# mit-han-lab/litepose

Measured on AMD Instinct MI355X. Metric: images/sec end-to-end (backbone+deconv+AE-group), LitePose-XS@256 b64, higher is better.
Workload: dtype f32

## Files before the change

litepose_amd/csrc/net_kernels.hip:

```cpp
#include "kernels.h"
#include "split3.h"

#include <cstdio>
#include <cstdlib>
#include <type_traits>
#include <utility>

namespace lp {

thread_local const char* last_kernel_tag = "";
thread_local LaunchNote last_launch;
thread_local bool launch_notes = false;

void note_launch(const void* fn, dim3 grid, dim3 block, size_t lds) {
    int per_cu = 0;
    const int threads = (int)(block.x * block.y * block.z);
    if (hipOccupancyMaxActiveBlocksPerMultiprocessor(&per_cu, fn, threads, lds) != hipSuccess) per_cu = 0;
    last_launch.grid = (int)((long)grid.x * grid.y * grid.z);
    last_launch.block = threads;
    last_launch.lds = (int)lds;
    last_launch.wgs_per_cu = per_cu;
}

typedef float f32x4 __attribute__((ext_vector_type(4)));
// ... 2234 lines not shown
        if (!mbconv2 || !wrow || !w1s || Cout > 16) return false;
        const size_t lds2 = (size_t)16 * MB3_PAIR * sizeof(float);
        last_kernel_tag = "mbconv2_kernel";
#define LP_MB2(RESV)                                                                                       \
        do {                                                                                               \
            if (uses_scratch(reinterpret_cast<const void*>(mbconv2_kernel<RESV, 8, 1>))) return false;     \
            static bool attr2_##RESV = false;                                                              \
            if (!attr2_##RESV) {                                                                           \
                (void)hipFuncSetAttribute(reinterpret_cast<const void*>(mbconv2_kernel<RESV, 8, 1>),       \
                                          hipFuncAttributeMaxDynamicSharedMemorySize, (int)lds2);          \
                attr2_##RESV = true;                                                                       \
            }                                                                                              \
            LP_LAUNCH((mbconv2_kernel<RESV, 8, 1>), grid, block, lds2, s, x, (const f32x4*)wrow,  \
                               (const u32x4*)w1s, b1f, w2p, b2f, out, Cin, Cexp, Cout, H, W, tilesX, tilesY, \
                               xcd_remap_mode());                                                          \
        } while (0)
        if (res) LP_MB2(true); else LP_MB2(false);
#undef LP_MB2
        return true;
    }
    const size_t lds = (size_t)(16 * MB2_PAIR) * sizeof(float);
    last_kernel_tag = "mbconv_kernel";
#define LP_MB(RESV)                                                                                        \
    do {                                                                                                   \
        if (uses_scratch(reinterpret_cast<const void*>(mbconv_kernel<RESV, 12, false, false>))) return false; \
        static bool attr_##RESV = false;                                                                   \
        if (!attr_##RESV) {                                                                                \
            (void)hipFuncSetAttribute(reinterpret_cast<const void*>(mbconv_kernel<RESV, 12, false, false>), \
                                      hipFuncAttributeMaxDynamicSharedMemorySize, (int)lds);               \
            attr_##RESV = true;                                                                            \
        }                                                                                                  \
        LP_LAUNCH((mbconv_kernel<RESV, 12, false, false>), grid, block, lds, s, x, (const f32x4*)nullptr, \
                           (const u32x4*)nullptr, w1p, b1f, wdw_pair, bdw, w2p, b2f, out, Cin, Cexp, Cout, H, W, \
                           tilesX, tilesY, xcd_remap_mode());                                              \
    } while (0)
    if (res) LP_MB(true); else LP_MB(false);
#undef LP_MB
    return true;
}

template <int COT, bool DUAL>
__global__ __launch_bounds__(256) void deconv_pair_kernel(const float* __restrict__ inA, int Ca,
                                                          const float* __restrict__ inB, int Cb,
                                                          const float* __restrict__ w,
                                                          const float* __restrict__ b,
                                                          float* __restrict__ out, int N, int h,
                                                          int w_, int Cout) {
    const long total = (long)N * h * w_;
    const long g = (long)blockIdx.x * blockDim.x + threadIdx.x;
    if (g >= total) return;
    const int ix = (int)(g % w_);
    const int iy = (int)((g / w_) % h);
    const int n = (int)(g / ((long)w_ * h));
    const int co0 = blockIdx.y * COT;
    float acc[COT][4];
#pragma unroll
    for (int c = 0; c < COT; ++c) acc[c][0] = acc[c][1] = acc[c][2] = acc[c][3] = 0.f;

    for (int src = 0; src < (DUAL ? 2 : 1); ++src) {
        const float* in = src == 0 ? inA : inB;
        const int Cs = src == 0 ? Ca : Cb;
        const int cbase = src == 0 ? 0 : Ca;
        for (int ci = 0; ci < Cs; ++ci) {
            const float* plane = in + ((long)n * Cs + ci) * h * w_;
            float v[3][3];
#pragma unroll
            for (int dy = -1; dy <= 1; ++dy)
#pragma unroll
                for (int dx = -1; dx <= 1; ++dx) {
                    const int y = iy + dy, x = ix + dx;
                    v[dy + 1][dx + 1] =
                        (y >= 0 && y < h && x >= 0 && x < w_) ? plane[(long)y * w_ + x] : 0.f;
                }
            const float* wc = w + ((long)(cbase + ci) * Cout + co0) * 16;
#pragma unroll
            for (int c = 0; c < COT; ++c) {
                if (co0 + c < Cout) {
                    const float* k = wc + c * 16;
#pragma unroll
                    for (int a = 0; a < 2; ++a)
#pragma unroll
                        for (int bb = 0; bb < 2; ++bb) {
                            const int dy0 = a == 0 ? 0 : 1, ky0 = a == 0 ? 1 : 0;
                            const int dy1 = a == 0 ? -1 : 0, ky1 = a == 0 ? 3 : 2;
                            const int dx0 = bb == 0 ? 0 : 1, kx0 = bb == 0 ? 1 : 0;
                            const int dx1 = bb == 0 ? -1 : 0, kx1 = bb == 0 ? 3 : 2;
                            float t = acc[c][a * 2 + bb];
                            t = fmaf(v[dy0 + 1][dx0 + 1], k[ky0 * 4 + kx0], t);
                            t = fmaf(v[dy0 + 1][dx1 + 1], k[ky0 * 4 + kx1], t);
                            t = fmaf(v[dy1 + 1][dx0 + 1], k[ky1 * 4 + kx0], t);
                            t = fmaf(v[dy1 + 1][dx1 + 1], k[ky1 * 4 + kx1], t);
                            acc[c][a * 2 + bb] = t;
                        }
                }
            }
        }
    }
    const int OW = 2 * w_, OH = 2 * h;
#pragma unroll
    for (int c = 0; c < COT; ++c) {
        const int co = co0 + c;
        if (co < Cout) {
            const float bias = b[co];
            float* o = out + ((long)n * Cout + co) * OH * OW + (long)(2 * iy) * OW + 2 * ix;
            float2 r0 = {fmaxf(acc[c][0] + bias, 0.f), fmaxf(acc[c][1] + bias, 0.f)};
            float2 r1 = {fmaxf(acc[c][2] + bias, 0.f), fmaxf(acc[c][3] + bias, 0.f)};
            *reinterpret_cast<float2*>(o) = r0;
            *reinterpret_cast<float2*>(o + OW) = r1;
        }
    }
}

template <bool DUAL>
__global__ __launch_bounds__(256) void deconv_mfma_kernel(const float* __restrict__ inA, int Ca,
                                                          const float* __restrict__ inB, int Cb,
                                                          const float* __restrict__ wp,
                                                          const float* __restrict__ bias,
                                                          float* __restrict__ out, long NP, int h, int w_,
                                                          int Cout) {
    const int lane = threadIdx.x & 63;
    const int wave = threadIdx.x >> 6;
    const long px0 = ((long)blockIdx.x * 4 + wave) * 32;
    if (px0 >= NP) return;
    const int half = lane >> 5, pl = lane & 31;
    const long g = px0 + pl;
    const bool valid = g < NP;
    const long gc = valid ? g : NP - 1;
    const int hw = h * w_;
    const int n = (int)(gc / hw);
    const int p = (int)(gc - (long)n * hw);
    const int iy = p / w_, ix = p - iy * w_;
    const int par = blockIdx.y, a = par >> 1, b = par & 1;
    const int Ct = DUAL ? Ca + Cb : Ca;
    const int KP = 2 * Ct;
    int toff[4];
    bool tok[4];
#pragma unroll
    for (int t = 0; t < 4; ++t) {
        const int tyi = t >> 1, txi = t & 1;
        const int dy = a == 0 ? (tyi == 0 ? 0 : -1) : (tyi == 0 ? 1 : 0);
        const int dx = b == 0 ? (txi == 0 ? 0 : -1) : (txi == 0 ? 1 : 0);
        const int y = iy + dy, x = ix + dx;
        tok[t] = y >= 0 && y < h && x >= 0 && x < w_;
        toff[t] = tok[t] ? y * w_ + x : p;
    }
    f32x16 acc;
#pragma unroll
    for (int r = 0; r < 16; ++r) acc[r] = 0.f;
    const f32x4* bp = reinterpret_cast<const f32x4*>(bias + half * 16);
    f32x4 bfr[4];
#pragma unroll
    for (int q = 0; q < 4; ++q) bfr[q] = bp[q];
    const float* wl = wp + (long)par * KP * 64 + lane;
    int kbase = 0;
#pragma unroll
    for (int t = 0; t < 4; ++t) {
#pragma unroll 1
        for (int srcsel = 0; srcsel < (DUAL ? 2 : 1); ++srcsel) {
            const int C = srcsel == 0 ? Ca : Cb;
            const float* sp = (srcsel == 0 ? inA : inB) + ((long)n * C + half) * hw + toff[t];
            const int nkp = C >> 1;
#pragma unroll 8
            for (int kp = 0; kp < nkp; ++kp) {
                float bv = sp[(long)(2 * kp) * hw];
                bv = tok[t] ? bv : 0.f;
                const float av = wl[(long)(kbase + kp) * 64];
                acc = __builtin_amdgcn_mfma_f32_32x32x2f32(av, bv, acc, 0, 0, 0);
            }
            kbase += nkp;
        }
    }
    if (!valid) return;
    const int OW = 2 * w_;
    float* ob = out + (long)n * Cout * 4 * hw + (long)(2 * iy + a) * OW + 2 * ix + b;
#pragma unroll
    for (int r = 0; r < 16; ++r) {
        const int co = 4 * half + (r & 3) + 8 * (r >> 2);
        if (co < Cout) ob[(long)co * 4 * hw] = fmaxf(acc[r] + bfr[r >> 2][r & 3], 0.f);
    }
}

template <int NB, bool DUAL>
__global__ __launch_bounds__(256) void deconv4_kernel(const float* __restrict__ inA, int Ca,
                                                      const float* __restrict__ inB, int Cb,
                                                      const f32x4* __restrict__ wq,
                                                      const float* __restrict__ bias,
                                                      float* __restrict__ out, long NP, int h, int w_,
                                                      int Cout, int xcd_remap) {
    const int lane = threadIdx.x & 63;
    const int wave = threadIdx.x >> 6;
    const int bid = xcd_remap ? xcd_contiguous_id(blockIdx.x, gridDim.x) : blockIdx.x;
    const long px0 = ((long)bid * 4 + wave) * 32;
    if (px0 >= NP) return;
    const int half = lane >> 5, pl = lane & 31;
    const long g = px0 + pl;
    const bool valid = g < NP;
    const long gc = valid ? g : NP - 1;
    const int hw = h * w_;
    const int n = (int)(gc / hw);
    const int p = (int)(gc - (long)n * hw);
    const int iy = p / w_, ix = p - iy * w_;
    int voff[9];
    bool vok[9];
#pragma unroll
    for (int v = 0; v < 9; ++v) {
        const int y = iy + v / 3 - 1, x = ix + v % 3 - 1;
        vok[v] = y >= 0 && y < h && x >= 0 && x < w_;
        voff[v] = vok[v] ? y * w_ + x : p;
    }
    f32x16 acc[NB][4];
#pragma unroll
    for (int i = 0; i < NB; ++i)
#pragma unroll
        for (int q = 0; q < 4; ++q)
#pragma unroll
            for (int r = 0; r < 16; ++r) acc[i][q][r] = 0.f;
    f32x4 bfr[NB][4];
#pragma unroll
    for (int i = 0; i < NB; ++i) {
        const f32x4* bp = reinterpret_cast<const f32x4*>(bias + (i * 2 + half) * 16);
#pragma unroll
        for (int q = 0; q < 4; ++q) bfr[i][q] = bp[q];
    }
    const int CP = (DUAL ? Ca + Cb : Ca) >> 1, CPA = Ca >> 1;
    const f32x4* wl = wq + lane;
    const float* spA = inA + ((long)n * Ca + half) * hw;
    const float* spB = DUAL ? inB + ((long)n * Cb + half) * hw : spA;
    auto fetch = [&](int cp, float (&bv)[9], f32x4 (&av)[NB][4]) {
        const int c = min(cp, CP - 1);
        const float* cpn = (!DUAL || c < CPA) ? spA + (long)(2 * c) * hw : spB + (long)(2 * (c - CPA)) * hw;
#pragma unroll
        for (int v = 0; v < 9; ++v) bv[v] = cpn[voff[v]];
#pragma unroll
        for (int i = 0; i < NB; ++i)
#pragma unroll
            for (int q = 0; q < 4; ++q) av[i][q] = wl[((long)(i * 4 + q) * CP + c) * 64];
    };
    auto mma = [&](const float (&raw)[9], const f32x4 (&av)[NB][4]) {
        float bv[9];
#pragma unroll
        for (int v = 0; v < 9; ++v) bv[v] = vok[v] ? raw[v] : 0.f;
#pragma unroll
        for (int t = 0; t < 4; ++t) {
            const int tyi = t >> 1, txi = t & 1;
#pragma unroll
            for (int i = 0; i < NB; ++i)
#pragma unroll
                for (int q = 0; q < 4; ++q) {
                    const int a = q >> 1, b = q & 1;
                    const int dy = a == 0 ? (tyi == 0 ? 0 : -1) : (tyi == 0 ? 1 : 0);
                    const int dx = b == 0 ? (txi == 0 ? 0 : -1) : (txi == 0 ? 1 : 0);
                    acc[i][q] = __builtin_amdgcn_mfma_f32_32x32x2f32(av[i][q][t], bv[(dy + 1) * 3 + dx + 1], acc[i][q],
                                                                     0, 0, 0);
                }
        }
    };
    float bv0[9], bv1[9];
    f32x4 av0[NB][4], av1[NB][4];
    fetch(0, bv0, av0);
#pragma unroll 1
    for (int cp = 0; cp < CP; cp += 2) {
        fetch(cp + 1, bv1, av1);
        __builtin_amdgcn_sched_barrier(0);
        mma(bv0, av0);
        __builtin_amdgcn_sched_barrier(0);
        fetch(cp + 2, bv0, av0);
        __builtin_amdgcn_sched_barrier(0);
        mma(bv1, av1);
        __builtin_amdgcn_sched_barrier(0);
    }
    if (!valid) return;
    const int OW = 2 * w_;
    float* ob = out + (long)n * Cout * 4 * hw + (long)(2 * iy) * OW + 2 * ix;
#pragma unroll
    for (int i = 0; i < NB; ++i)
#pragma unroll
        for (int r = 0; r < 16; ++r) {
            const int co = i * 32 + 4 * half + (r & 3) + 8 * (r >> 2);
            if (co < Cout) {
                const float bb = bfr[i][r >> 2][r & 3];
                float* o = ob + (long)co * 4 * hw;
                const float2 top = {fmaxf(acc[i][0][r] + bb, 0.f), fmaxf(acc[i][1][r] + bb, 0.f)};
                const float2 bot = {fmaxf(acc[i][2][r] + bb, 0.f), fmaxf(acc[i][3][r] + bb, 0.f)};
                *reinterpret_cast<float2*>(o) = top;
                *reinterpret_cast<float2*>(o + OW) = bot;
            }
        }
}

void launch_deconv4(const float* inA, int Ca, const float* inB, int Cb, const float* wq, const float* bias,
                    float* out, int N, int h, int w_, int Cout, hipStream_t s) {
    const long NP = (long)N * h * w_;
    dim3 grid((unsigned)((NP + 127) / 128)), block(256);
#define LP_D4(NBV, DV) LP_LAUNCH((deconv4_kernel<NBV, DV>), grid, block, 0, s, inA, Ca, inB, Cb, (const f32x4*)wq, bias, \
                                 out, NP, h, w_, Cout, xcd_remap_mode())
    if (inB) { if (Cout <= 32) LP_D4(1, true); else LP_D4(2, true); }
    else { if (Cout <= 32) LP_D4(1, false); else LP_D4(2, false); }
#undef LP_D4
    last_kernel_tag = "deconv4_kernel";
}


struct D4X3 {
    __host__ __device__ static constexpr int twl(int w) { return w <= 16 ? 4 : 5; }
    __host__ __device__ static constexpr int rows(int twl) { return 4 * (32 >> twl); }
    __host__ __device__ static constexpr int rs(int twl) { return twl == 5 ? 34 : 32; }
    __host__ __device__ static constexpr int cells(int twl) { return (rows(twl) + 2) * rs(twl); }
    __host__ __device__ static constexpr int slab_groups(int twl) { return twl == 5 ? 6 : 4; }
    static constexpr int REC = 48;
};

struct D4Prod { int v, q, t; };
__host__ __device__ constexpr D4Prod d4x3_prod(int p) {
    int k = 0;
    for (int v = 0; v < 9; ++v)
        for (int q = 0; q < 4; ++q)
            for (int t = 0; t < 4; ++t) {
                const int a = q >> 1, b = q & 1, tyi = t >> 1, txi = t & 1;
                const int dy = a == 0 ? (tyi == 0 ? 0 : -1) : (tyi == 0 ? 1 : 0);
                const int dx = b == 0 ? (txi == 0 ? 0 : -1) : (txi == 0 ? 1 : 0);
                if (dy == v / 3 - 1 && dx == v % 3 - 1) {
                    if (k == p) return {v, q, t};
                    ++k;
                }
            }
    return {0, 0, 0};
}
template <class F, int... U>
__device__ __forceinline__ void d4x3_units(F&& f, std::integer_sequence<int, U...>) {
    (f(std::integral_constant<int, U>{}), ...);
}

template <int NB, bool DUAL>
__global__ __launch_bounds__(256, NB == 1 ? 3 : 2) void deconv4x3_kernel(
    const float* __restrict__ inA, int Ca, const float* __restrict__ inB, int Cb, const u32x4* __restrict__ ws,
    const float* __restrict__ bias, float* __restrict__ out, int tilesX, int tilesY, int h, int w_, int Cout,
    int SG, int xcd_remap) {
    extern __shared__ __attribute__((aligned(16))) unsigned char d4s[];
    const int lane = threadIdx.x & 63;
    const int wave = threadIdx.x >> 6;
    const int bid = xcd_remap ? xcd_contiguous_id(blockIdx.x, gridDim.x) : blockIdx.x;
    const int twl = D4X3::twl(w_), TW = 1 << twl, RS = D4X3::rs(twl), HW2 = TW + 2;
    const int NCELL = D4X3::cells(twl);
    const int CPG = (D4X3::rows(twl) + 2) * HW2;
    const int tpi = tilesX * tilesY;
    const int n = bid / tpi, t = bid - n * tpi;
    const int ty = t / tilesX, tx = t - ty * tilesX;
    const int y0 = ty * D4X3::rows(twl), x0 = tx * TW;
    const int half = lane >> 5, pl = lane & 31;
    const int ry = wave * (32 >> twl) + (pl >> twl), cx = pl & (TW - 1);
    const int iy = y0 + ry, ix = x0 + cx;
    const bool valid = iy < h && ix < w_;
    const bool wave_live = y0 + wave * (32 >> twl) < h;
    const int hw = h * w_;
    f32x16 acc[NB][4];
#pragma unroll
    for (int i = 0; i < NB; ++i)
#pragma unroll
        for (int q = 0; q < 4; ++q)
#pragma unroll
            for (int r = 0; r < 16; ++r) acc[i][q][r] = 0.f;
    const int Ga = Ca >> 3, G8 = (DUAL ? Ca + Cb : Ca) >> 3, KS = (G8 + 1) >> 1;
    const float* baseA = inA + (long)n * Ca * hw;
    const float* baseB = DUAL ? inB + (long)n * Cb * hw : baseA;
    const unsigned char* cell = d4s + ((ry + 1) * RS + cx + 1) * D4X3::REC;
    constexpr int UN = 16 * NB, DEPTH = NB == 1 ? 2 : 4;
    u32x4 ar[DEPTH][3];
    auto fetch_a = [&](int ksn, auto uc) {
        constexpr int u = decltype(uc)::value, i = u % NB;
        constexpr D4Prod pr = d4x3_prod(u / NB);
        const u32x4* wp = ws + ((long)((i * 4 + pr.q) * 4 + pr.t) * KS + ksn) * 3 * 64;
        ar[u % DEPTH][0] = wp[lane];
        ar[u % DEPTH][1] = wp[64 + lane];
        ar[u % DEPTH][2] = wp[128 + lane];
    };
    constexpr int U = 4;
#pragma unroll 1
    for (int g0 = 0; g0 < G8; g0 += SG) {
        const int ng = min(SG, G8 - g0), items = ng * CPG;
        if (g0) __syncthreads();
#pragma unroll 1
        for (int it = threadIdx.x; it < items; it += 256 * U) {
            float raw[U][8];
            int dst[U];
            bool ok[U];
#pragma unroll
            for (int u = 0; u < U; ++u) {
                const int e = min(it + 256 * u, items - 1);
                const int gl = e / CPG, c = e - gl * CPG;
                const int r = c / HW2, x = c - r * HW2;
                const int gy = y0 - 1 + r, gx = x0 - 1 + x;
                ok[u] = gy >= 0 && gy < h && gx >= 0 && gx < w_;
                const int gq = g0 + gl;
                const float* sp = (!DUAL || gq < Ga) ? baseA + (long)(8 * gq) * hw : baseB + (long)(8 * (gq - Ga)) * hw;
                sp += ok[u] ? gy * w_ + gx : 0;
                dst[u] = (gl * NCELL + r * RS + x) * D4X3::REC;
#pragma unroll
                for (int ch = 0; ch < 8; ++ch) raw[u][ch] = sp[(long)ch * hw];
            }
#pragma unroll
            for (int u = 0; u < U; ++u) {
                u32x4 fh, fm, fl;
#pragma unroll
                for (int j = 0; j < 4; ++j) {
                    const Split3 s3 = split3_pair(ok[u] ? raw[u][2 * j] : 0.f, ok[u] ? raw[u][2 * j + 1] : 0.f);
                    fh[j] = s3.h;
                    fm[j] = s3.m;
                    fl[j] = s3.l;
                }
                u32x4* rec = reinterpret_cast<u32x4*>(d4s + dst[u]);
                rec[0] = fh;
                rec[1] = fm;
                rec[2] = fl;
            }
        }
        if (g0 == 0) {
            d4x3_units([&](auto uc) { fetch_a(0, uc); }, std::make_integer_sequence<int, DEPTH - 1>{});
        }
        __syncthreads();
        if (!wave_live) continue;
        const int ks1 = (g0 + ng + 1) >> 1;
#pragma unroll 1
        for (int ks = g0 >> 1; ks < ks1; ++ks) {
            const int gl = min(2 * ks + half, G8 - 1) - g0;
            const unsigned char* kc = cell + gl * NCELL * D4X3::REC;
            const int ksn = min(ks + 1, KS - 1);
            u32x4 bf[2][3];
            auto view = [&](int v, u32x4 (&b)[3]) {
                const u32x4* rec = reinterpret_cast<const u32x4*>(kc + ((v / 3 - 1) * RS + v % 3 - 1) * D4X3::REC);
                b[0] = rec[0];
                b[1] = rec[1];
                b[2] = rec[2];
            };
            view(0, bf[0]);
            d4x3_units([&](auto uc) {
                constexpr int u = decltype(uc)::value, pi = u / NB, i = u % NB;
                constexpr D4Prod pr = d4x3_prod(pi);
                constexpr bool first = i == 0 && (pi == 0 || d4x3_prod(pi - 1).v != pr.v);
                if constexpr (u + DEPTH - 1 < UN) fetch_a(ks, std::integral_constant<int, u + DEPTH - 1>{});
                else fetch_a(ksn, std::integral_constant<int, u + DEPTH - 1 - UN>{});
                if constexpr (first && pr.v < 8) view(pr.v + 1, bf[(pr.v + 1) & 1]);
                __builtin_amdgcn_sched_barrier(0);
                acc[i][pr.q] = mma6(ar[u % DEPTH], bf[pr.v & 1][0], bf[pr.v & 1][1], bf[pr.v & 1][2], acc[i][pr.q]);
                __builtin_amdgcn_sched_barrier(0);
            }, std::make_integer_sequence<int, UN>{});
        }
    }
    if (!valid) return;
    const int OW = 2 * w_;
    float* ob = out + (long)n * Cout * 4 * hw + (long)(2 * iy) * OW + 2 * ix;
#pragma unroll
    for (int i = 0; i < NB; ++i) {
        const f32x4* bp = reinterpret_cast<const f32x4*>(bias + (i * 2 + half) * 16);
#pragma unroll
        for (int r = 0; r < 16; ++r) {
            const int co = i * 32 + 4 * half + (r & 3) + 8 * (r >> 2);
            if (co < Cout) {
                const float bb = bp[r >> 2][r & 3];
                float* o = ob + (long)co * 4 * hw;
                const float2 top = {fmaxf(acc[i][0][r] + bb, 0.f), fmaxf(acc[i][1][r] + bb, 0.f)};
                const float2 bot = {fmaxf(acc[i][2][r] + bb, 0.f), fmaxf(acc[i][3][r] + bb, 0.f)};
                *reinterpret_cast<float2*>(o) = top;
                *reinterpret_cast<float2*>(o + OW) = bot;
            }
        }
    }
}

bool launch_deconv4x3(const float* inA, int Ca, const float* inB, int Cb, const void* ws, const float* bias,
                      float* out, int N, int h, int w_, int Cout, hipStream_t s) {
    if (!ws || (Ca & 7) || (Cb & 7) || Cout > 64) return false;
    if (h * w_ <= 256) return false;
    const int twl = D4X3::twl(w_), G8 = (Ca + (inB ? Cb : 0)) >> 3;
    const int tilesX = (w_ + (1 << twl) - 1) >> twl, tilesY = (h + D4X3::rows(twl) - 1) / D4X3::rows(twl);
    const int nslab = (G8 + D4X3::slab_groups(twl) - 1) / D4X3::slab_groups(twl);
    const int SG = (((G8 + nslab - 1) / nslab) + 1) & ~1;
    const size_t lds = (size_t)(G8 < SG ? G8 : SG) * D4X3::cells(twl) * D4X3::REC;
    dim3 grid((unsigned)((long)N * tilesX * tilesY)), block(256);
#define LP_D4X3(NBV, DV) LP_LAUNCH((deconv4x3_kernel<NBV, DV>), grid, block, lds, s, inA, Ca, inB, Cb, (const u32x4*)ws, bias, \
                                   out, tilesX, tilesY, h, w_, Cout, SG, xcd_remap_mode())
    if (inB) { if (Cout <= 32) LP_D4X3(1, true); else LP_D4X3(2, true); }
    else { if (Cout <= 32) LP_D4X3(1, false); else LP_D4X3(2, false); }
#undef LP_D4X3
    last_kernel_tag = "deconv4x3_kernel";
    return true;
}

void launch_deconv_mfma(const float* inA, int Ca, const float* inB, int Cb, const float* wp,
                        const float* bias, float* out, int N, int h, int w_, int Cout, hipStream_t s) {
    const long NP = (long)N * h * w_;
    dim3 grid((unsigned)((NP + 127) / 128), 4), block(256);
    if (inB)
        LP_LAUNCH(deconv_mfma_kernel<true>, grid, block, 0, s, inA, Ca, inB, Cb, wp, bias, out, NP, h, w_, Cout);
    else
        LP_LAUNCH(deconv_mfma_kernel<false>, grid, block, 0, s, inA, Ca, inB, Cb, wp, bias, out, NP, h, w_, Cout);
    last_kernel_tag = "deconv_mfma_kernel";
}

void launch_deconv_pair(const float* inA, int Ca, const float* inB, int Cb, const float* w,
                        const float* b, float* out, int N, int h, int w_, int Cout, hipStream_t s) {
    constexpr int COT = 8;
    const long total = (long)N * h * w_;
    dim3 grid((unsigned)((total + 255) / 256), (Cout + COT - 1) / COT), block(256);
    if (inB)
        LP_LAUNCH((deconv_pair_kernel<COT, true>), grid, block, 0, s, inA, Ca, inB, Cb, w, b, out, N, h, w_, Cout);
    else
        LP_LAUNCH((deconv_pair_kernel<COT, false>), grid, block, 0, s, inA, Ca, inB, Cb, w, b, out, N, h, w_, Cout);
    last_kernel_tag = "deconv_pair_kernel";
}

}
```

litepose_amd/csrc/split3.h:

```cpp
#pragma once
#include <hip/hip_runtime.h>

namespace lp {

typedef float f32x2 __attribute__((ext_vector_type(2)));
typedef float f32x4 __attribute__((ext_vector_type(4)));
typedef float f32x16 __attribute__((ext_vector_type(16)));
typedef short bf16x8_t __attribute__((ext_vector_type(8)));
typedef unsigned u32x4 __attribute__((ext_vector_type(4)));

__device__ __forceinline__ void keep_b128(f32x4& v) { asm("" : "+v"(v)); }

struct Split3 { unsigned h, m, l; };
__device__ __forceinline__ Split3 split3_pair(float x0, float x1) {
    const unsigned u0 = __float_as_uint(x0), u1 = __float_as_uint(x1);
    const float r0 = x0 - __uint_as_float(u0 & 0xffff0000u);
    const float r1 = x1 - __uint_as_float(u1 & 0xffff0000u);
    const unsigned m0 = __float_as_uint(r0), m1 = __float_as_uint(r1);
    const float s0 = r0 - __uint_as_float(m0 & 0xffff0000u);
    const float s1 = r1 - __uint_as_float(m1 & 0xffff0000u);
    Split3 r;
    r.h = __builtin_amdgcn_perm(u1, u0, 0x07060302u);
    r.m = __builtin_amdgcn_perm(m1, m0, 0x07060302u);
    r.l = __builtin_amdgcn_perm(__float_as_uint(s1), __float_as_uint(s0), 0x07060302u);
    return r;
}

__device__ __forceinline__ f32x16 mma6(const u32x4 (&a)[3], const u32x4& bh, const u32x4& bm, const u32x4& bl,
                                       f32x16 acc) {
#define LP_M(AT, BV)                                                                           \
    acc = __builtin_amdgcn_mfma_f32_32x32x16_bf16(__builtin_bit_cast(bf16x8_t, a[AT]),          \
                                                  __builtin_bit_cast(bf16x8_t, BV), acc, 0, 0, 0)
    LP_M(2, bh);
    LP_M(0, bl);
    LP_M(1, bm);
    LP_M(1, bh);
    LP_M(0, bm);
    LP_M(0, bh);
#undef LP_M
    return acc;
}

}
```

Measured before the change: 22990.

## Double deconv4x3 row tile for narrow outputs to reuse weight fragments

For the Cout<=32 variant, each wave now covers two row blocks (CB=2), so one loaded weight fragment feeds two sets of MFMAs via a new mma6x2 helper. The goal is to halve weight global/L2 traffic per output and raise MFMA density. LDS slabs are resized to half a CU's LDS, with the dynamic shared memory limit raised, and launch bounds drop to 2 waves-groups per CU. The trade-off is more accumulator registers, larger LDS tiles, fewer blocks in the grid, and lower occupancy.

```diff
diff --git a/litepose_amd/csrc/net_kernels.hip b/litepose_amd/csrc/net_kernels.hip
--- a/litepose_amd/csrc/net_kernels.hip
+++ b/litepose_amd/csrc/net_kernels.hip
@@ -2560,13 +2560,29 @@
 
 
 struct D4X3 {
+    __host__ __device__ static constexpr int cb(int nb) { return nb == 1 ? 2 : 1; }
     __host__ __device__ static constexpr int twl(int w) { return w <= 16 ? 4 : 5; }
-    __host__ __device__ static constexpr int rows(int twl) { return 4 * (32 >> twl); }
+    __host__ __device__ static constexpr int rows(int twl, int cb) { return 4 * cb * (32 >> twl); }
     __host__ __device__ static constexpr int rs(int twl) { return twl == 5 ? 34 : 32; }
-    __host__ __device__ static constexpr int cells(int twl) { return (rows(twl) + 2) * rs(twl); }
-    __host__ __device__ static constexpr int slab_groups(int twl) { return twl == 5 ? 6 : 4; }
+    __host__ __device__ static constexpr int cells(int twl, int cb) { return (rows(twl, cb) + 2) * rs(twl); }
     static constexpr int REC = 48;
+    static constexpr int LDS_HALF_CU = 160 * 1024 / 2;
+    __host__ __device__ static constexpr int slab_groups(int twl, int cb) {
+        return cb == 1 ? (twl == 5 ? 6 : 4) : LDS_HALF_CU / (cells(twl, cb) * REC);
+    }
+    __host__ __device__ static constexpr int slab(int G8, int twl, int cb) {
+        const int mx = slab_groups(twl, cb), me = mx & ~1;
+        const int nslab = G8 <= mx ? 1 : (G8 + me - 1) / me;
+        return (((G8 + nslab - 1) / nslab) + 1) & ~1;
+    }
+    __host__ __device__ static constexpr int lds_bytes(int G8, int twl, int cb) {
+        const int sg = slab(G8, twl, cb);
+        return (G8 < sg ? G8 : sg) * cells(twl, cb) * REC;
+    }
 };
+static_assert(D4X3::slab_groups(5, 2) == 5 && D4X3::slab_groups(4, 2) == 2 && D4X3::slab(5, 5, 2) == 6 &&
+              D4X3::slab(6, 5, 2) == 4 && D4X3::slab(7, 5, 2) == 4 && D4X3::slab(17, 5, 1) == 6 && D4X3::slab(7, 5, 1) == 4,
+              "deconv4x3 slab rule");
 
 struct D4Prod { int v, q, t; };
 __host__ __device__ constexpr D4Prod d4x3_prod(int p) {
@@ -2590,7 +2606,7 @@
 }
 
 template <int NB, bool DUAL>
-__global__ __launch_bounds__(256, NB == 1 ? 3 : 2) void deconv4x3_kernel(
+__global__ __launch_bounds__(256, 2) void deconv4x3_kernel(
     const float* __restrict__ inA, int Ca, const float* __restrict__ inB, int Cb, const u32x4* __restrict__ ws,
     const float* __restrict__ bias, float* __restrict__ out, int tilesX, int tilesY, int h, int w_, int Cout,
     int SG, int xcd_remap) {
@@ -2598,30 +2614,33 @@
     const int lane = threadIdx.x & 63;
     const int wave = threadIdx.x >> 6;
     const int bid = xcd_remap ? xcd_contiguous_id(blockIdx.x, gridDim.x) : blockIdx.x;
-    const int twl = D4X3::twl(w_), TW = 1 << twl, RS = D4X3::rs(twl), HW2 = TW + 2;
-    const int NCELL = D4X3::cells(twl);
-    const int CPG = (D4X3::rows(twl) + 2) * HW2;
+    constexpr int CB = D4X3::cb(NB);
+    const int twl = D4X3::twl(w_), TW = 1 << twl, RS = D4X3::rs(twl), HW2 = TW + 2, RW = 32 >> twl;
+    const int NCELL = D4X3::cells(twl, CB);
+    const int CPG = (D4X3::rows(twl, CB) + 2) * HW2;
     const int tpi = tilesX * tilesY;
     const int n = bid / tpi, t = bid - n * tpi;
     const int ty = t / tilesX, tx = t - ty * tilesX;
-    const int y0 = ty * D4X3::rows(twl), x0 = tx * TW;
+    const int y0 = ty * D4X3::rows(twl, CB), x0 = tx * TW;
     const int half = lane >> 5, pl = lane & 31;
-    const int ry = wave * (32 >> twl) + (pl >> twl), cx = pl & (TW - 1);
+    const int ry = wave * CB * RW + (pl >> twl), cx = pl & (TW - 1);
     const int iy = y0 + ry, ix = x0 + cx;
-    const bool valid = iy < h && ix < w_;
-    const bool wave_live = y0 + wave * (32 >> twl) < h;
+    const bool wave_live = y0 + wave * CB * RW < h;
     const int hw = h * w_;
-    f32x16 acc[NB][4];
-#pragma unroll
-    for (int i = 0; i < NB; ++i)
-#pragma unroll
-        for (int q = 0; q < 4; ++q)
-#pragma unroll
-            for (int r = 0; r < 16; ++r) acc[i][q][r] = 0.f;
+    f32x16 acc[CB][NB][4];
+#pragma unroll
+    for (int c = 0; c < CB; ++c)
+#pragma unroll
+        for (int i = 0; i < NB; ++i)
+#pragma unroll
+            for (int q = 0; q < 4; ++q)
+#pragma unroll
+                for (int r = 0; r < 16; ++r) acc[c][i][q][r] = 0.f;
     const int Ga = Ca >> 3, G8 = (DUAL ? Ca + Cb : Ca) >> 3, KS = (G8 + 1) >> 1;
     const float* baseA = inA + (long)n * Ca * hw;
     const float* baseB = DUAL ? inB + (long)n * Cb * hw : baseA;
     const unsigned char* cell = d4s + ((ry + 1) * RS + cx + 1) * D4X3::REC;
+    const int blk = RW * RS * D4X3::REC;
     constexpr int UN = 16 * NB, DEPTH = NB == 1 ? 2 : 4;
     u32x4 ar[DEPTH][3];
     auto fetch_a = [&](int ksn, auto uc) {
@@ -2683,12 +2702,16 @@
             const int gl = min(2 * ks + half, G8 - 1) - g0;
             const unsigned char* kc = cell + gl * NCELL * D4X3::REC;
             const int ksn = min(ks + 1, KS - 1);
-            u32x4 bf[2][3];
-            auto view = [&](int v, u32x4 (&b)[3]) {
-                const u32x4* rec = reinterpret_cast<const u32x4*>(kc + ((v / 3 - 1) * RS + v % 3 - 1) * D4X3::REC);
-                b[0] = rec[0];
-                b[1] = rec[1];
-                b[2] = rec[2];
+            u32x4 bf[2][CB][3];
+            auto view = [&](int v, u32x4 (&b)[CB][3]) {
+#pragma unroll
+                for (int c = 0; c < CB; ++c) {
+                    const u32x4* rec =
+                        reinterpret_cast<const u32x4*>(kc + c * blk + ((v / 3 - 1) * RS + v % 3 - 1) * D4X3::REC);
+                    b[c][0] = rec[0];
+                    b[c][1] = rec[1];
+                    b[c][2] = rec[2];
+                }
             };
             view(0, bf[0]);
             d4x3_units([&](auto uc) {
@@ -2699,27 +2722,35 @@
                 else fetch_a(ksn, std::integral_constant<int, u + DEPTH - 1 - UN>{});
                 if constexpr (first && pr.v < 8) view(pr.v + 1, bf[(pr.v + 1) & 1]);
                 __builtin_amdgcn_sched_barrier(0);
-                acc[i][pr.q] = mma6(ar[u % DEPTH], bf[pr.v & 1][0], bf[pr.v & 1][1], bf[pr.v & 1][2], acc[i][pr.q]);
+                if constexpr (CB == 2)
+                    mma6x2(ar[u % DEPTH], bf[pr.v & 1][0], bf[pr.v & 1][1], acc[0][i][pr.q], acc[1][i][pr.q]);
+                else
+                    acc[0][i][pr.q] = mma6(ar[u % DEPTH], bf[pr.v & 1][0][0], bf[pr.v & 1][0][1], bf[pr.v & 1][0][2],
+                                           acc[0][i][pr.q]);
                 __builtin_amdgcn_sched_barrier(0);
             }, std::make_integer_sequence<int, UN>{});
         }
     }
-    if (!valid) return;
     const int OW = 2 * w_;
-    float* ob = out + (long)n * Cout * 4 * hw + (long)(2 * iy) * OW + 2 * ix;
-#pragma unroll
-    for (int i = 0; i < NB; ++i) {
-        const f32x4* bp = reinterpret_cast<const f32x4*>(bias + (i * 2 + half) * 16);
-#pragma unroll
-        for (int r = 0; r < 16; ++r) {
-            const int co = i * 32 + 4 * half + (r & 3) + 8 * (r >> 2);
-            if (co < Cout) {
-                const float bb = bp[r >> 2][r & 3];
-                float* o = ob + (long)co * 4 * hw;
-                const float2 top = {fmaxf(acc[i][0][r] + bb, 0.f), fmaxf(acc[i][1][r] + bb, 0.f)};
-                const float2 bot = {fmaxf(acc[i][2][r] + bb, 0.f), fmaxf(acc[i][3][r] + bb, 0.f)};
-                *reinterpret_cast<float2*>(o) = top;
-                *reinterpret_cast<float2*>(o + OW) = bot;
+#pragma unroll
+    for (int c = 0; c < CB; ++c) {
+        const int oy = iy + c * RW;
+        if (oy >= h || ix >= w_) continue;
+        float* ob = out + (long)n * Cout * 4 * hw + (long)(2 * oy) * OW + 2 * ix;
+#pragma unroll
+        for (int i = 0; i < NB; ++i) {
+            const f32x4* bp = reinterpret_cast<const f32x4*>(bias + (i * 2 + half) * 16);
+#pragma unroll
+            for (int r = 0; r < 16; ++r) {
+                const int co = i * 32 + 4 * half + (r & 3) + 8 * (r >> 2);
+                if (co < Cout) {
+                    const float bb = bp[r >> 2][r & 3];
+                    float* o = ob + (long)co * 4 * hw;
+                    const float2 top = {fmaxf(acc[c][i][0][r] + bb, 0.f), fmaxf(acc[c][i][1][r] + bb, 0.f)};
+                    const float2 bot = {fmaxf(acc[c][i][2][r] + bb, 0.f), fmaxf(acc[c][i][3][r] + bb, 0.f)};
+                    *reinterpret_cast<float2*>(o) = top;
+                    *reinterpret_cast<float2*>(o + OW) = bot;
+                }
             }
         }
     }
@@ -2729,12 +2760,21 @@
                       float* out, int N, int h, int w_, int Cout, hipStream_t s) {
     if (!ws || (Ca & 7) || (Cb & 7) || Cout > 64) return false;
     if (h * w_ <= 256) return false;
-    const int twl = D4X3::twl(w_), G8 = (Ca + (inB ? Cb : 0)) >> 3;
-    const int tilesX = (w_ + (1 << twl) - 1) >> twl, tilesY = (h + D4X3::rows(twl) - 1) / D4X3::rows(twl);
-    const int nslab = (G8 + D4X3::slab_groups(twl) - 1) / D4X3::slab_groups(twl);
-    const int SG = (((G8 + nslab - 1) / nslab) + 1) & ~1;
-    const size_t lds = (size_t)(G8 < SG ? G8 : SG) * D4X3::cells(twl) * D4X3::REC;
+    const int twl = D4X3::twl(w_), G8 = (Ca + (inB ? Cb : 0)) >> 3, cb = D4X3::cb(Cout <= 32 ? 1 : 2);
+    const int rows = D4X3::rows(twl, cb);
+    const int tilesX = (w_ + (1 << twl) - 1) >> twl, tilesY = (h + rows - 1) / rows;
+    const int SG = D4X3::slab(G8, twl, cb);
+    const size_t lds = (size_t)D4X3::lds_bytes(G8, twl, cb);
     dim3 grid((unsigned)((long)N * tilesX * tilesY)), block(256);
+    static bool attr = false;
+    if (!attr) {
+        const int mx = D4X3::LDS_HALF_CU;
+        (void)hipFuncSetAttribute(reinterpret_cast<const void*>(deconv4x3_kernel<1, true>),
+                                  hipFuncAttributeMaxDynamicSharedMemorySize, mx);
+        (void)hipFuncSetAttribute(reinterpret_cast<const void*>(deconv4x3_kernel<1, false>),
+                                  hipFuncAttributeMaxDynamicSharedMemorySize, mx);
+        attr = true;
+    }
 #define LP_D4X3(NBV, DV) LP_LAUNCH((deconv4x3_kernel<NBV, DV>), grid, block, lds, s, inA, Ca, inB, Cb, (const u32x4*)ws, bias, \
                                    out, tilesX, tilesY, h, w_, Cout, SG, xcd_remap_mode())
     if (inB) { if (Cout <= 32) LP_D4X3(1, true); else LP_D4X3(2, true); }
diff --git a/litepose_amd/csrc/split3.h b/litepose_amd/csrc/split3.h
--- a/litepose_amd/csrc/split3.h
+++ b/litepose_amd/csrc/split3.h
@@ -41,4 +41,20 @@
     return acc;
 }
 
+__device__ __forceinline__ void mma6x2(const u32x4 (&a)[3], const u32x4 (&b0)[3], const u32x4 (&b1)[3], f32x16& acc0,
+                                       f32x16& acc1) {
+#define LP_M2(AT, BP)                                                                                              \
+    acc0 = __builtin_amdgcn_mfma_f32_32x32x16_bf16(__builtin_bit_cast(bf16x8_t, a[AT]),                             \
+                                                   __builtin_bit_cast(bf16x8_t, b0[BP]), acc0, 0, 0, 0);            \
+    acc1 = __builtin_amdgcn_mfma_f32_32x32x16_bf16(__builtin_bit_cast(bf16x8_t, a[AT]),                             \
+                                                   __builtin_bit_cast(bf16x8_t, b1[BP]), acc1, 0, 0, 0)
+    LP_M2(2, 0);
+    LP_M2(0, 2);
+    LP_M2(1, 1);
+    LP_M2(1, 0);
+    LP_M2(0, 1);
+    LP_M2(0, 0);
+#undef LP_M2
 }
+
+}
```

Result: no change. 22970 (-0.1%).
